# hjsuh94/irs_mpc

Hardware: AMD Instinct MI355X
Metric: rollouts*timesteps/s (randomized-smoothing pass) + iLQR-iters/s (higher is better)
Workload: dtype f32; 1 GPU; planar_hand quasi-dynamic contact, zero-order-B smoothing, step QP solved exactly (dual active-set method) -- the metric's config; T=50, N_per_gpu=10000, N_total=10000, mode=ZERO_ORDER_B, contact_solver=exact, samples=supplied, resident in HBM (f32), parallelism=samples sharded over 1 GPU(s), 1 all-reduce of (T,P) f64 per step

## Files before the change

### irs_mpc_amd/csrc/smooth_ug.hip

```cpp
#include "smooth_common.hpp"

namespace {

#ifndef IRS_UG_SWEEPS
#define IRS_UG_SWEEPS 6
#endif
#ifndef IRS_UG_PDAS
#define IRS_UG_PDAS 4
#endif
#ifndef IRS_UG_BLOCK
#define IRS_UG_BLOCK 512
#endif
constexpr int kUgBlock = IRS_UG_BLOCK;
constexpr int kUgSweeps = IRS_UG_SWEEPS;
constexpr int kUgPdas = IRS_UG_PDAS;
constexpr int kUgTabStride = 76;
#ifndef IRS_UG_NOM_ROUNDS
#define IRS_UG_NOM_ROUNDS 2
#endif
constexpr int kUgNomRounds = IRS_UG_NOM_ROUNDS;
constexpr int kUgRing = 128;

template <class Model>
struct alignas(16) UgLds {
    static constexpr int NC = Model::NC, n = Model::NX, m = Model::NU;
    float tab[1 << NC][kUgTabStride];
    float W[NC][NC];
    float invw[NC];
    float Wd[NC];
    float r0[NC];
    float phi[NC];
    float C[m][NC];
    float JD[n][NC];
    float Jc[NC][n];
    float Dinv[n];
    float Db0[n];
    float DK[m];
    float q[n];
};

__device__ __forceinline__ float ug_uniform(float v) {
    return __int_as_float(__builtin_amdgcn_readfirstlane(__float_as_int(v)));
}

template <int NC>
struct UgUni {
    float W[NC * (NC + 1) / 2];
    float invw[NC];
    float r0[NC];
    __device__ __forceinline__ float w(int i, int j) const {
        return i <= j ? W[i * NC - i * (i - 1) / 2 + (j - i)] : W[j * NC - j * (j - 1) / 2 + (i - j)];
    }
};

template <class Model>
__device__ __forceinline__ unsigned ug_lookup(const UgLds<Model>& S, unsigned a, const float* x, float tol, float* v,
                                              float* tau) {
    constexpr int NC = Model::NC;
    static_assert(NC == 8, "table entries are 8 x 8");
    const float4* e = reinterpret_cast<const float4*>(&S.tab[a][0]);
    float4 g4[2 * NC + 2];
#pragma unroll
    for (int c = 0; c < 2 * NC + 2; ++c) g4[c] = e[c];
    const unsigned ap = __float_as_uint(S.tab[a][72]);
    tau[0] = g4[16].x; tau[1] = g4[16].y; tau[2] = g4[16].z; tau[3] = g4[16].w;
    tau[4] = g4[17].x; tau[5] = g4[17].y; tau[6] = g4[17].z; tau[7] = g4[17].w;
#pragma unroll
    for (int i = 0; i < NC; ++i) v[i] = tau[i] * tol;
#pragma unroll
    for (int c = 0; c < NC; ++c) {
        const float4 lo = g4[2 * c], hi = g4[2 * c + 1];
        v[0] = fmaf(lo.x, x[c], v[0]); v[1] = fmaf(lo.y, x[c], v[1]);
        v[2] = fmaf(lo.z, x[c], v[2]); v[3] = fmaf(lo.w, x[c], v[3]);
        v[4] = fmaf(hi.x, x[c], v[4]); v[5] = fmaf(hi.y, x[c], v[5]);
        v[6] = fmaf(hi.z, x[c], v[6]); v[7] = fmaf(hi.w, x[c], v[7]);
    }
    return ap;
}

template <class Model>
__device__ __forceinline__ float ug_rhs(const UgUni<Model::NC>& U, const UgLds<Model>& S, const float* du, float* r) {
    constexpr int NC = Model::NC, m = Model::NU;
#pragma unroll
    for (int c = 0; c < NC; ++c) r[c] = U.r0[c];
#pragma unroll
    for (int j = 0; j < m; ++j) {
        const float4 lo = *reinterpret_cast<const float4*>(&S.C[j][0]);
        const float4 hi = *reinterpret_cast<const float4*>(&S.C[j][4]);
        r[0] = fmaf(lo.x, du[j], r[0]); r[1] = fmaf(lo.y, du[j], r[1]);
        r[2] = fmaf(lo.z, du[j], r[2]); r[3] = fmaf(lo.w, du[j], r[3]);
        r[4] = fmaf(hi.x, du[j], r[4]); r[5] = fmaf(hi.y, du[j], r[5]);
        r[6] = fmaf(hi.z, du[j], r[6]); r[7] = fmaf(hi.w, du[j], r[7]);
    }
    float scale = 1e-30f;
#pragma unroll
    for (int c = 0; c < NC; ++c) scale = fmaxf(scale, fabsf(r[c]));
    return 1e-6f * scale;
}

template <class Model>
__device__ __forceinline__ bool ug_try(const UgUni<Model::NC>& U, const UgLds<Model>& S, const float* r, float tolv,
                                       float* lam, unsigned& a_out, int diag = 0) {
    constexpr int NC = Model::NC;
    float g[NC];
#pragma unroll
    for (int i = 0; i < NC; ++i) { lam[i] = 0.f; g[i] = r[i]; }
#pragma unroll 2
    for (int sw = 0; sw < ((diag & 64) ? 0 : kUgSweeps); ++sw) {
#pragma unroll
        for (int i = 0; i < NC; ++i) {
            const float nw = fmaxf(fmaf(-g[i], U.invw[i], lam[i]), 0.f);
            const float dl = nw - lam[i];
            lam[i] = nw;
#pragma unroll
            for (int j = 0; j < NC; ++j) g[j] = fmaf(U.w(j, i), dl, g[j]);
        }
    }
    unsigned a = 0u;
#pragma unroll
    for (int i = 0; i < NC; ++i) a |= (lam[i] > 0.f) ? (1u << i) : 0u;
    bool done = (diag & 32) != 0;
    for (int it = 0; it < kUgPdas; ++it) {
        float v[NC], tau[NC];
        const unsigned ap = ug_lookup<Model>(S, a, r, tolv, v, tau);
        unsigned bad = 0u;
#pragma unroll
        for (int i = NC - 1; i >= 0; --i) bad = __builtin_amdgcn_alignbit(bad, __float_as_uint(v[i]), 31);
        if (!done) {
            if (bad == 0u) {
#pragma unroll
                for (int i = 0; i < NC; ++i) lam[i] = fmaf(-tau[i], v[i], v[i]);
                done = true;
            }
            a = ap ^ bad;
        }
        if (__all(done)) break;
    }
    a_out = a;
    return done;
}

template <class Model>
__device__ __forceinline__ void ug_full(const UgLds<Model>& S, const float* r, float tolv, unsigned a, float* lam,
                                        int cap = 4 * Model::NC) {
    constexpr int NC = Model::NC;
    constexpr float kBig = 3.0e38f, piv_rel = 1e-5f;
    float g[NC];
    bool valid = false;
    for (int round = 0; round < 3; ++round) {
        if (__all(valid)) break;
        float v[NC], tau[NC];
        const unsigned ap = ug_lookup<Model>(S, a, r, 0.f, v, tau);
        if (!valid) {
            unsigned negb = 0u;
#pragma unroll
            for (int i = 0; i < NC; ++i) {
                const bool in = tau[i] == 0.f;
                negb |= (in && !(v[i] > 0.f)) ? (1u << i) : 0u;
                lam[i] = in ? v[i] : 0.f;
                g[i] = in ? 0.f : v[i];
            }
            valid = negb == 0u;
            a = ap & ~negb;
        }
    }
    if (!valid) {
        a = 0u;
#pragma unroll
        for (int i = 0; i < NC; ++i) { lam[i] = 0.f; g[i] = r[i]; }
    }
    int p = -1;
    bool done = false;
    for (int it = 0; it < cap; ++it) {
        if (!done && p < 0) {
            float vmin = kBig;
            int c = 0;
#pragma unroll
            for (int i = 0; i < NC; ++i) {
                const float vv = ((a >> i) & 1u) ? kBig : g[i];
                if (vv < vmin) { vmin = vv; c = i; }
            }
            if (vmin >= -tolv) done = true;
            else p = c;
        }
        if (__all(done)) break;
        const int pp = (done || p < 0) ? 0 : p;
        float wp[NC], u[NC], tau[NC];
        {
            const float4 lo = *reinterpret_cast<const float4*>(&S.W[pp][0]);
            const float4 hi = *reinterpret_cast<const float4*>(&S.W[pp][4]);
            wp[0] = lo.x; wp[1] = lo.y; wp[2] = lo.z; wp[3] = lo.w;
            wp[4] = hi.x; wp[5] = hi.y; wp[6] = hi.z; wp[7] = hi.w;
        }
        ug_lookup<Model>(S, a, wp, 0.f, u, tau);
        const float wpp = S.Wd[pp];
        float gp = 0.f, zp = 0.f;
#pragma unroll
        for (int i = 0; i < NC; ++i) {
            const bool isp = i == pp;
            gp = isp ? g[i] : gp;
            zp = isp ? u[i] : zp;
        }
        const bool full_ok = zp > piv_rel * wpp;
        const float t2 = full_ok ? -gp * irs_rcp_fast(zp) : kBig;
        float rho[NC], qv[NC];
        float t1 = kBig;
#pragma unroll
        for (int i = 0; i < NC; ++i) {
            rho[i] = fmaf(tau[i], u[i], -u[i]);
            qv[i] = rho[i] > 0.f ? lam[i] * irs_rcp_fast(rho[i]) : kBig;
            t1 = fminf(t1, qv[i]);
        }
        int kb = 0;
#pragma unroll
        for (int i = NC - 1; i >= 0; --i) kb = (qv[i] == t1) ? i : kb;
        const float tmin = fminf(t1, t2);
        if (!done && !(tmin < kBig)) done = true;
        const float tt = done ? 0.f : tmin;
#pragma unroll
        for (int i = 0; i < NC; ++i) {
            g[i] = fmaf(tt * tau[i], u[i], g[i]);
            lam[i] = fmaxf(fmaf(-tt, rho[i], lam[i]) + ((i == pp) ? tt : 0.f), 0.f);
        }
        if (!done) {
            const bool full = t2 <= t1;
            if (full) {
                a |= 1u << pp;
                p = -1;
            } else {
                a &= ~(1u << kb);
#pragma unroll
                for (int i = 0; i < NC; ++i) lam[i] = (i == kb) ? 0.f : lam[i];
            }
        }
    }
}

template <class Model>
__device__ __forceinline__ void ug_build_entry(UgLds<Model>& S, unsigned a, int half) {
    constexpr int NC = Model::NC;
    constexpr float piv_rel = 1e-5f;
    float M_[NC][NC], inv[NC], W[NC][NC];
    bool act[NC];
#pragma unroll
    for (int i = 0; i < NC; ++i) {
        act[i] = ((a >> i) & 1u) != 0u;
#pragma unroll
        for (int j = 0; j < NC; ++j) W[i][j] = S.W[i][j];
#pragma unroll
        for (int j = 0; j <= i; ++j) M_[i][j] = W[i][j];
    }
    unsigned ap = 0u;
#pragma unroll
    for (int j = 0; j < NC; ++j) {
        const float dj = M_[j][j];
        const bool ok = act[j] && dj > piv_rel * W[j][j];
        act[j] = ok;
        ap |= ok ? (1u << j) : 0u;
        inv[j] = ok ? irs_rcp_fast(dj) : 0.f;
#pragma unroll
        for (int i = j + 1; i < NC; ++i) M_[j][i] = M_[i][j] * inv[j];
#pragma unroll
        for (int i = j + 1; i < NC; ++i)
#pragma unroll
            for (int k = j + 1; k <= i; ++k) M_[i][k] = M_[i][k] - M_[j][i] * M_[k][j];
    }
    float* e = &S.tab[a][0];
    for (int cc = 0; cc < NC / 2; ++cc) {
        const int c = half * (NC / 2) + cc;
        float y[NC];
#pragma unroll
        for (int j = 0; j < NC; ++j) {
            float v = (act[j] && j == c) ? -1.f : 0.f;
#pragma unroll
            for (int k = 0; k < j; ++k) v = v - M_[k][j] * y[k];
            y[j] = v;
        }
#pragma unroll
        for (int j = NC - 1; j >= 0; --j) {
            float v = y[j] * inv[j];
#pragma unroll
            for (int i = j + 1; i < NC; ++i) v = v - M_[j][i] * y[i];
            y[j] = v;
        }
        float col[NC];
#pragma unroll
        for (int i = 0; i < NC; ++i) {
            float s = (i == c) ? 1.f : 0.f;
#pragma unroll
            for (int j = 0; j < NC; ++j) s = fmaf(W[i][j], y[j], s);
            col[i] = act[i] ? y[i] : s;
        }
        *reinterpret_cast<float4*>(e + 8 * c) = make_float4(col[0], col[1], col[2], col[3]);
        *reinterpret_cast<float4*>(e + 8 * c + 4) = make_float4(col[4], col[5], col[6], col[7]);
    }
    if (half == 0) {
        *reinterpret_cast<float4*>(e + 64) = make_float4(act[0] ? 0.f : 1.f, act[1] ? 0.f : 1.f, act[2] ? 0.f : 1.f, act[3] ? 0.f : 1.f);
        *reinterpret_cast<float4*>(e + 68) = make_float4(act[4] ? 0.f : 1.f, act[5] ? 0.f : 1.f, act[6] ? 0.f : 1.f, act[7] ? 0.f : 1.f);
        e[72] = __uint_as_float(ap);
    }
}

struct UgNomLds {
    double J[8][7];
    double q[7], Dinv[7], b[7];
};

template <class Model>
__device__ __forceinline__ double ug_nominal_geometry(const SmoothArgs& a, UgNomLds& L, int t, int lane) {
    constexpr int NC = Model::NC, n = Model::NX, m = Model::NU;
    double x64[n], u64[m], q[n], Dinv[n], b[n], J[NC][n], phi[NC];
#pragma unroll
    for (int i = 0; i < n; ++i) x64[i] = a.x_trj[(size_t)t * n + i];
#pragma unroll
    for (int j = 0; j < m; ++j) u64[j] = a.u_trj[(size_t)t * m + j];
    Model::template assemble<double>(a.p, x64, u64, q, Dinv, b, J, phi);
    if (lane == 0) {
#pragma unroll
        for (int c = 0; c < NC; ++c)
#pragma unroll
            for (int k = 0; k < n; ++k) L.J[c][k] = J[c][k];
#pragma unroll
        for (int k = 0; k < n; ++k) { L.q[k] = q[k]; L.Dinv[k] = Dinv[k]; L.b[k] = b[k]; }
    }
    double rr = 0.0;
#pragma unroll
    for (int c = 0; c < NC; ++c) {
        double s = phi[c];
#pragma unroll
        for (int k = 0; k < n; ++k) s -= J[c][k] * (b[k] * Dinv[k]);
        rr = (lane == c) ? s : rr;
    }
    wave_sync();
    return rr;
}

template <class Model>
__device__ __forceinline__ void ug_nominal(const SmoothArgs& a, const UgUni<Model::NC>& U, const UgLds<Model>& S,
                                           UgNomLds& L, double rr, int t, int lane) {
    constexpr int NC = Model::NC, n = Model::NX, m = Model::NU;
    static_assert(NC == 8 && n <= 8, "lane (i,k) = 8 i + k owns entry (i,k) of the 8 x 8 dual Hessian");
    float du0[m], r32[NC], lam32[NC];
#pragma unroll
    for (int j = 0; j < m; ++j) du0[j] = 0.f;
    const float tolv = ug_rhs<Model>(U, S, du0, r32);
    unsigned am = 0u;
    if (!ug_try<Model>(U, S, r32, tolv, lam32, am)) ug_full<Model>(S, r32, tolv, am, lam32);
    unsigned set = 0u;
#pragma unroll
    for (int i = 0; i < NC; ++i) set |= (lam32[i] > 0.f) ? (1u << i) : 0u;
    set = (unsigned)__builtin_amdgcn_readfirstlane((int)set);
    {
        const int li = lane >> 3, lk = lane & 7;
        double w = 0.0;
#pragma unroll
        for (int kk = 0; kk < n; ++kk) w += L.J[li][kk] * L.Dinv[kk] * L.J[lk][kk];
        double scale = 1e-300;
#pragma unroll
        for (int c = 0; c < NC; ++c) scale = fmax(scale, fabs(__shfl(rr, c, 64)));
        const double tol64 = 1e-10 * scale;
        double lamd = 0.0;
        bool settled = false;
        for (int corr = 0; corr < 8 && !settled; ++corr) {
            double M = w, Lf = 0.0;
            unsigned eff = 0u;
            double invd[NC];
#pragma unroll
            for (int j = 0; j < NC; ++j) {
                const double dj = __shfl(M, 9 * j, 64), wjj = __shfl(w, 9 * j, 64);
                const bool ok = ((set >> j) & 1u) && dj > 1e-7 * wjj;
                eff |= ok ? (1u << j) : 0u;
                invd[j] = ok ? 1.0 / dj : 0.0;
                const double Mij = __shfl(M, 8 * li + j, 64), Mkj = __shfl(M, 8 * lk + j, 64);
                if (lk == j && li > j) Lf = Mij * invd[j];
                if (li > j && lk > j) M -= Mij * invd[j] * Mkj;
            }
            const bool mine = lane < NC && ((eff >> lane) & 1u);
            double y = mine ? -rr : 0.0;
#pragma unroll
            for (int j = 0; j < NC; ++j) {
                const double yj = __shfl(y, j, 64);
                const double Lij = __shfl(Lf, 8 * (lane & 7) + j, 64);
                if (lane < NC && lane > j) y -= Lij * yj;
            }
            double invme = 0.0;
#pragma unroll
            for (int j = 0; j < NC; ++j) invme = (lane == j) ? invd[j] : invme;
            y *= invme;
#pragma unroll
            for (int j = NC - 1; j >= 0; --j) {
                const double yj = __shfl(y, j, 64);
                const double Lji = __shfl(Lf, 8 * j + (lane & 7), 64);
                if (lane < j) y -= Lji * yj;
            }
            lamd = mine ? y : 0.0;
            double pr = w * __shfl(lamd, lk, 64);
            pr += __shfl_xor(pr, 1, 64);
            pr += __shfl_xor(pr, 2, 64);
            pr += __shfl_xor(pr, 4, 64);
            const double sl = rr + __shfl(pr, 8 * (lane & 7), 64);
            const bool neg = lane < NC && mine && !(lamd > 0.0);
            const bool viol = lane < NC && !mine && sl < -tol64;
            const unsigned negb = (unsigned)(__ballot(neg) & 0xffull), violb = (unsigned)(__ballot(viol) & 0xffull);
            if ((negb | violb) == 0u) settled = true;
            else set = (eff & ~negb) | violb;
        }
        double f = 0.0;
        if (settled) {
            double acc = 0.0;
#pragma unroll
            for (int c = 0; c < NC; ++c) acc += L.J[c][lane < n ? lane : 0] * __shfl(lamd, c, 64);
            if (lane < n) f = L.q[lane] + L.Dinv[lane] * (acc - L.b[lane]);
        } else if (lane < n) {
            float acc = -S.Db0[lane];
#pragma unroll
            for (int c = 0; c < NC; ++c) acc = fmaf(S.JD[lane][c], lam32[c], acc);
            f = (double)(S.q[lane] + acc);
        }
        if (lane < n)
            __hip_atomic_store(a.fnom + (size_t)t * n + Model::perm(lane), f, __ATOMIC_RELAXED, __HIP_MEMORY_SCOPE_AGENT);
    }
}

#ifdef IRS_UG_STAMPS
constexpr int kUgStampSlots = 12, kUgStampWgs = 2048;
__device__ unsigned long long ug_stamps[kUgStampWgs * kUgStampSlots];
#define UG_STAMP(slot)                                                                          \
    do {                                                                                        \
        if ((threadIdx.x & 63) == 0) {                                                          \
            const int wg_ = blockIdx.y * gridDim.x + blockIdx.x;                                \
            if (wg_ < kUgStampWgs && ((slot) < 8 ? threadIdx.x == 0 : true))                    \
                ug_stamps[wg_ * kUgStampSlots + (slot)] = __builtin_amdgcn_s_memtime();         \
        }                                                                                       \
    } while (0)
#else
#define UG_STAMP(slot) do {} while (0)
#endif

template <class Model, int MODE, bool RNG, bool FUSE>
__global__ __launch_bounds__(kUgBlock) void smooth_ug_kernel(SmoothArgs a) {
    using TR = SmoothTraits<Model, MODE>;
    constexpr int n = TR::n, m = TR::m, P = TR::P, NC = Model::NC;
    constexpr int BLOCK = kUgBlock, NW = BLOCK / 64;
    static_assert(TR::Z0 == n && NC == 8 && m == 4, "u-only smoothing of an 8-row contact model with 4 commands");
    static_assert(P < kBlock, "the hand-off's group reduction");
    constexpr int NG = m * (m + 1) / 2;
    constexpr int PI = TR::FIRST_B ? 1 : NG + m * NC + m;
    constexpr int PPI = irs_reduce_pad(TR::FIRST_B ? n * m : PI);
    constexpr int QE = m + 1;
    __shared__ UgLds<Model> S;
    __shared__ UgNomLds nomL;
    __shared__ float ring_all[NW * kUgRing * QE];
    __shared__ float red[NW * (PPI > TR::PP ? PPI : TR::PP)];
    __shared__ float toti[PPI];
    __shared__ unsigned hist[TR::FIRST_B ? (1 << NC) : 1];
    __shared__ double red64[TR::NGRP * P];
    __shared__ double tot[P];
    __shared__ FinalizeLds<Model, MODE> fin;
    __shared__ int s_ticket;

    const int t = blockIdx.y, blk = blockIdx.x, tid = threadIdx.x;
    const int lane = tid & 63, wave = tid >> 6;

    UG_STAMP(0);
    const bool nominal_wave = blk == 0 && wave == NW - 1;
    double nom_r = 0.0;
    if (nominal_wave && !(a.diag & 2)) nom_r = ug_nominal_geometry<Model>(a, nomL, t, lane);
    if (wave == 0) {
        float xb[n], ub[m], q[n], Dinv[n], b0[n], J[NC][n], phi[NC];
#pragma unroll
        for (int i = 0; i < n; ++i) xb[i] = (float)a.x_trj[(size_t)t * n + i];
#pragma unroll
        for (int j = 0; j < m; ++j) ub[j] = (float)a.u_trj[(size_t)t * m + j];
        Model::template assemble<float>(a.p, xb, ub, q, Dinv, b0, J, phi);
        if (lane == 0) {
#pragma unroll
            for (int i = 0; i < NC; ++i) {
                S.phi[i] = phi[i];
#pragma unroll
                for (int k = 0; k < n; ++k) S.Jc[i][k] = J[i][k];
            }
#pragma unroll
            for (int k = 0; k < n; ++k) { S.Db0[k] = b0[k] * Dinv[k]; S.q[k] = q[k]; S.Dinv[k] = Dinv[k]; }
#pragma unroll
            for (int j = 0; j < m; ++j) S.DK[j] = Dinv[Model::act(j)] * Model::template stiffness<float>(a.p, j);
        }
    }
    if constexpr (TR::FIRST_B) {
        for (int q = tid; q < (1 << NC); q += BLOCK) hist[q] = 0u;
    }
    __syncthreads();
    if (tid < NC * NC) {
        const int i = tid / NC, j = tid % NC, hi = i > j ? i : j, lo = i > j ? j : i;
        float w = (S.Jc[hi][0] * S.Dinv[0]) * S.Jc[lo][0];
#pragma unroll
        for (int k = 1; k < n; ++k) w = w + (S.Jc[hi][k] * S.Dinv[k]) * S.Jc[lo][k];
        S.W[i][j] = w;
        if (i == j) {
            S.Wd[i] = w;
            S.invw[i] = (float)kContactPgsOmega * irs_rcp_fast(w);
        }
    } else if (tid < NC * NC + NC) {
        const int i = tid - NC * NC;
        float ri = S.phi[i];
#pragma unroll
        for (int k = 0; k < n; ++k) ri = ri - S.Jc[i][k] * S.Db0[k];
        S.r0[i] = ri;
    } else if (tid < 2 * NC * NC + NC) {
        const int e = tid - (NC * NC + NC), k = e / NC, c = e % NC;
        if (k < n) S.JD[k][c] = S.Jc[c][k] * S.Dinv[k];
    } else if (tid < 2 * NC * NC + NC + m * NC) {
        const int e = tid - (2 * NC * NC + NC), j = e / NC, c = e % NC;
        S.C[j][c] = (S.Jc[c][Model::act(j)] * S.Dinv[Model::act(j)]) * Model::template stiffness<float>(a.p, j);
    }
    __syncthreads();
    UG_STAMP(1);
    if (!(a.diag & 4))
        for (int e = tid; e < 2 * (1 << NC); e += BLOCK) ug_build_entry<Model>(S, (unsigned)(e >> 1), e & 1);
    __syncthreads();

    UG_STAMP(2);
    UgUni<NC> U;
    {
        int q = 0;
#pragma unroll
        for (int i = 0; i < NC; ++i)
#pragma unroll
            for (int j = i; j < NC; ++j) U.W[q++] = S.W[i][j];
#pragma unroll
        for (int i = 0; i < NC; ++i) { U.invw[i] = S.invw[i]; U.r0[i] = S.r0[i]; }
    }

    float acc[PPI];
#pragma unroll
    for (int i = 0; i < PPI; ++i) acc[i] = 0.f;

    if (nominal_wave && !(a.diag & 2)) ug_nominal<Model>(a, U, S, nomL, nom_r, t, lane);
    if (nominal_wave) UG_STAMP(8);
    if (!(a.diag & 8)) {
        const int V = a.nblk * NW;
        const int me = nominal_wave ? V - 1 : (blk == 0 ? wave : blk * NW - 1 + wave);
        const int nblocks = (a.N + 63) / 64;
        int round = nominal_wave ? kUgNomRounds : 0;
        auto block_of = [&](int k) { return k < kUgNomRounds ? k * (V - 1) + me : kUgNomRounds * (V - 1) + (k - kUgNomRounds) * V + me; };
        float* ring = ring_all + wave * (kUgRing * QE);
        int qhead = 0, qtail = 0;
        int bk = block_of(round);
        float du_next[m];
#pragma unroll
        for (int j = 0; j < m; ++j) du_next[j] = 0.f;
        auto request = [&](int block) {
            if constexpr (!RNG) {
                if (block < nblocks) {
                    const int sidx = block * 64 + lane;
                    const size_t row = (size_t)t * a.N + (sidx < a.N ? sidx : a.N - 1);
                    load_row<m>(a.du + row * m, du_next);
                }
            }
        };
        request(bk);
        while (true) {
            const bool fresh = bk < nblocks;
            const int pending = qtail - qhead;
            const bool flush = pending >= 64 || (!fresh && pending > 0);
            if (!fresh && !flush) break;
            float du[m], r[NC], lam[NC];
            bool on, fin_ = true;
            if (flush) {
                __builtin_amdgcn_fence(__ATOMIC_RELEASE, "wavefront");
                __builtin_amdgcn_wave_barrier();
                __builtin_amdgcn_fence(__ATOMIC_ACQUIRE, "wavefront");
                const int take = min(64, pending);
                on = lane < take;
                const int slot = (qhead + (on ? lane : 0)) & (kUgRing - 1);
#pragma unroll
                for (int j = 0; j < m; ++j) du[j] = ring[slot * QE + j];
                const unsigned wm = __float_as_uint(ring[slot * QE + m]);
                const float tolv = ug_rhs<Model>(U, S, du, r);
                ug_full<Model>(S, r, tolv, wm, lam, (a.diag & 128) ? 8 : ((a.diag & 256) ? 12 : 4 * NC));
                qhead += take;
            } else {
                const int sidx = bk * 64 + lane;
                on = sidx < a.N;
                if constexpr (RNG) {
                    const unsigned long long gidx = a.sample_offset + (unsigned long long)sidx;
#pragma unroll
                    for (int j = n / 4; j < (n + m + 3) / 4; ++j) {
                        float g4[4];
                        philox_normal4(gidx, (unsigned)t, (unsigned)j, a.iter, a.seed, g4);
#pragma unroll
                        for (int c = 0; c < 4; ++c) {
                            const int idx = 4 * j + c;
                            if (idx >= n && idx < n + m) du[idx - n] = __fmul_rn(g4[c], a.std[idx]);
                        }
                    }
                } else {
#pragma unroll
                    for (int j = 0; j < m; ++j) du[j] = du_next[j];
                    request(block_of(round + 1));
                }
                const float tolv = ug_rhs<Model>(U, S, du, r);
                unsigned mask = 0u;
                fin_ = ug_try<Model>(U, S, r, tolv, lam, mask, a.diag);
                if (a.diag & 16) fin_ = true;
                const bool hard = on && !fin_;
                const unsigned long long bal = __ballot(hard);
                if (hard) {
                    const int slot = (qtail + __popcll(bal & ((1ull << lane) - 1ull))) & (kUgRing - 1);
#pragma unroll
                    for (int j = 0; j < m; ++j) ring[slot * QE + j] = du[j];
                    ring[slot * QE + m] = __uint_as_float(mask);
                }
                qtail += __popcll(bal);
                bk = block_of(++round);
            }
            const bool use = on && fin_;
            bool nonfinite = false;
#pragma unroll
            for (int j = 0; j < m; ++j) nonfinite = nonfinite || irs_nonfinite_bits(du[j]);
            if constexpr (TR::FIRST_B) {
                unsigned I = 0u;
#pragma unroll
                for (int i = 0; i < NC; ++i) I |= (lam[i] * S.Wd[i] > (float)kContactActiveTol) ? (1u << i) : 0u;
                if (use) __hip_atomic_fetch_add(&hist[I], 1u, __ATOMIC_RELAXED, __HIP_MEMORY_SCOPE_WORKGROUP);
                if (on && nonfinite) acc[0] = irs_poison();
            } else {
                float zz[m];
#pragma unroll
                for (int j = 0; j < m; ++j) zz[j] = use ? du[j] : 0.f;
                int q = 0;
#pragma unroll
                for (int i = 0; i < m; ++i)
#pragma unroll
                    for (int j = i; j < m; ++j) { acc[q] = fmaf(zz[i], zz[j], acc[q]); ++q; }
#pragma unroll
                for (int i = 0; i < m; ++i)
#pragma unroll
                    for (int c = 0; c < NC; ++c) { acc[q] = fmaf(zz[i], lam[c], acc[q]); ++q; }
#pragma unroll
                for (int i = 0; i < m; ++i) { acc[q] += zz[i]; ++q; }
                if (on && nonfinite) acc[0] = irs_poison();
            }
        }
    }

    UG_STAMP(3);
    if (blk == 0 && wave == 1) UG_STAMP(9);
    if constexpr (TR::FIRST_B) {
        __syncthreads();
        unsigned poison_bits = __float_as_uint(acc[0]);
        asm volatile("" : "+v"(poison_bits));
#pragma unroll
        for (int i = 0; i < PPI; ++i) acc[i] = 0.f;
        for (int I = tid; I < (1 << NC); I += BLOCK) {
            const unsigned cnt = hist[I];
            if (cnt == 0u) continue;
            const float* e = &S.tab[I][0];
            const unsigned ap = __float_as_uint(e[72]);
            float Y[NC][m];
#pragma unroll
            for (int i = 0; i < NC; ++i) {
                const bool in = ((ap >> i) & 1u) != 0u;
#pragma unroll
                for (int c = 0; c < m; ++c) {
                    float s = 0.f;
#pragma unroll
                    for (int j = 0; j < NC; ++j) s = fmaf(e[8 * j + i], S.Jc[j][Model::act(c)], s);
                    Y[i][c] = in ? -s : 0.f;
                }
            }
#pragma unroll
            for (int k = 0; k < n; ++k)
#pragma unroll
                for (int c = 0; c < m; ++c) {
                    float s = 0.f;
#pragma unroll
                    for (int i = 0; i < NC; ++i) s = fmaf(S.Jc[i][k], Y[i][c], s);
                    const float Bkc = (k == Model::act(c) ? 1.f : 0.f) - S.Dinv[k] * s;
                    acc[Model::perm(k) * m + c] += (float)cnt * Bkc;
                }
        }
        if ((poison_bits & 0x7f800000u) == 0x7f800000u) acc[0] = irs_poison();
        block_reduce_lds<P, NW>(acc, red);
    } else {
        block_reduce_lds<PI, NW>(acc, red);
        __syncthreads();
        for (int q = tid; q < PI; q += BLOCK) {
            float s = red[q];
#pragma unroll
            for (int w = 1; w < NW; ++w) s += red[w * PPI + q];
            toti[q] = s;
        }
        __syncthreads();
        float out = 0.f;
        if (tid < P) {
            if (tid < NG) out = toti[tid];
            else if (tid < NG + m * n) {
                const int i = (tid - NG) / n, kext = (tid - NG) % n;
                int k = 0, jact = -1;
#pragma unroll
                for (int kk = 0; kk < n; ++kk) k = (Model::perm(kk) == kext) ? kk : k;
#pragma unroll
                for (int j = 0; j < m; ++j) jact = (Model::act(j) == k) ? j : jact;
                float s = -S.Db0[k] * toti[NG + m * NC + i];
                for (int c = 0; c < NC; ++c) s = fmaf(S.JD[k][c], toti[NG + i * NC + c], s);
                if (jact >= 0) {
                    const int lo = i < jact ? i : jact, hi = i < jact ? jact : i;
                    s = fmaf(S.DK[jact], toti[lo * m - lo * (lo - 1) / 2 + (hi - lo)], s);
                }
                out = s;
            } else {
                out = toti[NG + m * NC + (tid - NG - m * n)];
            }
        }
        __syncthreads();
        for (int q = tid; q < NW * TR::PP; q += BLOCK) red[q] = 0.f;
        __syncthreads();
        if (tid < P) red[tid] = out;
    }
    UG_STAMP(4);
    smooth_finish<Model, MODE, FUSE, BLOCK, true>(a, red, red64, tot, fin, s_ticket, t, blk, tid, a.fnom + (size_t)t * n);
    UG_STAMP(5);
}

template <class Model, int MODE>
void ug_launch_m(const SmoothArgs& a, bool rng, bool fuse, hipStream_t st) {
    dim3 grid(a.nblk, a.T), block(kUgBlock);
    if (rng) {
        if (fuse) hipLaunchKernelGGL((smooth_ug_kernel<Model, MODE, true, true>), grid, block, 0, st, a);
        else hipLaunchKernelGGL((smooth_ug_kernel<Model, MODE, true, false>), grid, block, 0, st, a);
    } else {
        if (fuse) hipLaunchKernelGGL((smooth_ug_kernel<Model, MODE, false, true>), grid, block, 0, st, a);
        else hipLaunchKernelGGL((smooth_ug_kernel<Model, MODE, false, false>), grid, block, 0, st, a);
    }
}

}

#ifdef IRS_UG_STAMPS
extern "C" int irs_debug_ug_stamps(unsigned long long* host_out, int n_wgs) {
    if (n_wgs > kUgStampWgs) n_wgs = kUgStampWgs;
    return (int)hipMemcpyFromSymbol(host_out, HIP_SYMBOL(ug_stamps), (size_t)n_wgs * kUgStampSlots * sizeof(unsigned long long));
}
#endif

bool irs_smooth_ug_supported(int model, int mode) {
    const char* e = getenv("IRS_UG");
    if (e != nullptr && atoi(e) == 0) return false;
    return model == IRS_MODEL_PLANAR_HAND_EXACT && (mode == IRS_SMOOTH_ZERO_ORDER_B || mode == IRS_SMOOTH_FIRST_ORDER);
}

int irs_smooth_ug_nblk(int T, int N) {
    static int cus = 0;
    if (cus == 0) {
        hipDeviceProp_t prop;
        int dev = 0;
        cus = (hipGetDevice(&dev) == hipSuccess && hipGetDeviceProperties(&prop, dev) == hipSuccess)
                  ? prop.multiProcessorCount : 256;
        if (cus < 1) cus = 256;
    }
    const int nblocks = (N + 63) / 64, NW = kUgBlock / 64;
    int nb = cus / (T < 1 ? 1 : T);
    if (nb < 1) nb = 1;
    const int by_work = (nblocks + 1 + NW - 1) / NW;
    if (nb > by_work) nb = by_work;
    return nb < 1 ? 1 : nb;
}

int irs_smooth_ug_launch(int model, int mode, const SmoothArgs& a, bool rng, bool fuse, hipStream_t st) {
    if (model != IRS_MODEL_PLANAR_HAND_EXACT) return IRS_ERR_UNSUPPORTED;
    if (mode == IRS_SMOOTH_ZERO_ORDER_B) ug_launch_m<PlanarHandExactModel, IRS_SMOOTH_ZERO_ORDER_B>(a, rng, fuse, st);
    else if (mode == IRS_SMOOTH_FIRST_ORDER) ug_launch_m<PlanarHandExactModel, IRS_SMOOTH_FIRST_ORDER>(a, rng, fuse, st);
    else return IRS_ERR_UNSUPPORTED;
    return IRS_OK;
}
```

Baseline: 13.17 billion rollouts*timesteps/s.

## Hand off straggler active-set solves to quad-lane cooperative finishing

Once only a few lanes (at most 16) are still iterating in the full dual active-set loop, their state (lambda, g, active mask, pivot, tolerance) is staged to LDS. Each remaining sample is then finished by a quad of four lanes that each own two constraint rows, using DPP quad reductions for the min and pick steps. This targets wave divergence, where a whole wave waits on a few slow lanes doing serial 8-row work. It adds LDS staging, extra wave syncs and a per-wave stage buffer. A diag bit can disable the hand-off and another can force every sample down the hard path.

```diff
diff --git a/irs_mpc_amd/csrc/smooth_ug.hip b/irs_mpc_amd/csrc/smooth_ug.hip
--- a/irs_mpc_amd/csrc/smooth_ug.hip
+++ b/irs_mpc_amd/csrc/smooth_ug.hip
@@ -140,9 +140,112 @@
     return done;
 }
 
+__device__ __forceinline__ float ug_row_ratio(float tau, float u, float lam, float& rho) {
+    rho = fmaf(tau, u, -u);
+    return rho > 0.f ? lam * irs_rcp_fast(rho) : 3.0e38f;
+}
+__device__ __forceinline__ void ug_row_step(float tt, float tau, float u, float rho, bool isp, float& g, float& lam) {
+    g = fmaf(tt * tau, u, g);
+    lam = fmaxf(fmaf(-tt, rho, lam) + (isp ? tt : 0.f), 0.f);
+}
+
+constexpr int kUgStageSlots = 16;
+constexpr int kUgStageStride = 20;
+
+template <int CTRL>
+__device__ __forceinline__ int ug_quad_perm(int v) {
+    return __builtin_amdgcn_update_dpp(0, v, CTRL, 0xf, 0xf, true);
+}
+__device__ __forceinline__ float ug_quad_min(float v) {
+    v = fminf(v, __int_as_float(ug_quad_perm<0xB1>(__float_as_int(v))));
+    return fminf(v, __int_as_float(ug_quad_perm<0x4E>(__float_as_int(v))));
+}
+__device__ __forceinline__ int ug_quad_min(int v) {
+    v = min(v, ug_quad_perm<0xB1>(v));
+    return min(v, ug_quad_perm<0x4E>(v));
+}
+__device__ __forceinline__ float ug_quad_pick(float v) {
+    v = v + __int_as_float(ug_quad_perm<0xB1>(__float_as_int(v)));
+    return v + __int_as_float(ug_quad_perm<0x4E>(__float_as_int(v)));
+}
+
 template <class Model>
+__device__ __forceinline__ void ug_finish_quads(const UgLds<Model>& S, float* stage, int nslots, int it, int cap, int lane) {
+    constexpr int NC = Model::NC;
+    static_assert(NC == 8, "four lanes of two rows each");
+    constexpr float kBig = 3.0e38f, piv_rel = 1e-5f;
+    const int q = lane >> 2, h = lane & 3, i0 = 2 * h, i1 = 2 * h + 1;
+    const bool have = q < nslots;
+    float* slot = stage + (have ? q : 0) * kUgStageStride;
+    const float2 l2 = *reinterpret_cast<const float2*>(slot + i0);
+    const float2 g2 = *reinterpret_cast<const float2*>(slot + NC + i0);
+    const float2 ap2 = *reinterpret_cast<const float2*>(slot + 2 * NC);
+    const float tolv = slot[2 * NC + 2];
+    float lam0 = l2.x, lam1 = l2.y, g0 = g2.x, g1 = g2.y;
+    unsigned a = __float_as_uint(ap2.x);
+    int p = __float_as_int(ap2.y);
+    bool done = !have;
+    for (; it < cap; ++it) {
+        if (!done && p < 0) {
+            const float vv0 = ((a >> i0) & 1u) ? kBig : g0, vv1 = ((a >> i1) & 1u) ? kBig : g1;
+            const float vmin = ug_quad_min(fminf(vv0, vv1));
+            const int c = ug_quad_min(vv0 == vmin ? i0 : (vv1 == vmin ? i1 : NC)) & (NC - 1);
+            if (vmin >= -tolv) done = true;
+            else p = c;
+        }
+        if (__all(done)) break;
+        const int pp = (done || p < 0) ? 0 : p;
+        float wp[NC];
+        {
+            const float4 lo = *reinterpret_cast<const float4*>(&S.W[pp][0]);
+            const float4 hi = *reinterpret_cast<const float4*>(&S.W[pp][4]);
+            wp[0] = lo.x; wp[1] = lo.y; wp[2] = lo.z; wp[3] = lo.w;
+            wp[4] = hi.x; wp[5] = hi.y; wp[6] = hi.z; wp[7] = hi.w;
+        }
+        const float* e = &S.tab[a][0];
+        float2 col[NC];
+#pragma unroll
+        for (int c = 0; c < NC; ++c) col[c] = *reinterpret_cast<const float2*>(e + 8 * c + i0);
+        const float2 tau2 = *reinterpret_cast<const float2*>(e + 64 + i0);
+        const float wpp = S.Wd[pp];
+        float u0 = tau2.x * 0.f, u1 = tau2.y * 0.f;
+#pragma unroll
+        for (int c = 0; c < NC; ++c) {
+            u0 = fmaf(col[c].x, wp[c], u0);
+            u1 = fmaf(col[c].y, wp[c], u1);
+        }
+        const bool mine = (pp >> 1) == h, odd = (pp & 1) != 0;
+        const float gp = ug_quad_pick(mine ? (odd ? g1 : g0) : 0.f);
+        const float zp = ug_quad_pick(mine ? (odd ? u1 : u0) : 0.f);
+        const bool full_ok = zp > piv_rel * wpp;
+        const float t2 = full_ok ? -gp * irs_rcp_fast(zp) : kBig;
+        float rho0, rho1;
+        const float qv0 = ug_row_ratio(tau2.x, u0, lam0, rho0), qv1 = ug_row_ratio(tau2.y, u1, lam1, rho1);
+        const float t1 = ug_quad_min(fminf(qv0, qv1));
+        const int kb = ug_quad_min(qv0 == t1 ? i0 : (qv1 == t1 ? i1 : NC)) & (NC - 1);
+        const float tmin = fminf(t1, t2);
+        if (!done && !(tmin < kBig)) done = true;
+        const float tt = done ? 0.f : tmin;
+        ug_row_step(tt, tau2.x, u0, rho0, i0 == pp, g0, lam0);
+        ug_row_step(tt, tau2.y, u1, rho1, i1 == pp, g1, lam1);
+        if (!done) {
+            if (t2 <= t1) {
+                a |= 1u << pp;
+                p = -1;
+            } else {
+                a &= ~(1u << kb);
+                lam0 = (i0 == kb) ? 0.f : lam0;
+                lam1 = (i1 == kb) ? 0.f : lam1;
+            }
+        }
+    }
+    if (have) *reinterpret_cast<float2*>(slot + i0) = make_float2(lam0, lam1);
+}
+
+template <class Model, bool STAGED = false>
 __device__ __forceinline__ void ug_full(const UgLds<Model>& S, const float* r, float tolv, unsigned a, float* lam,
-                                        int cap = 4 * Model::NC) {
+                                        int cap = 4 * Model::NC, bool on = true, bool one_lane = true,
+                                        float* stage = nullptr, int lane = 0) {
     constexpr int NC = Model::NC;
     constexpr float kBig = 3.0e38f, piv_rel = 1e-5f;
     float g[NC];
@@ -170,8 +273,10 @@
         for (int i = 0; i < NC; ++i) { lam[i] = 0.f; g[i] = r[i]; }
     }
     int p = -1;
-    bool done = false;
-    for (int it = 0; it < cap; ++it) {
+    bool done = STAGED ? !on : false;
+    int it = 0;
+    unsigned long long hand = 0ull;
+    for (; it < cap; ++it) {
         if (!done && p < 0) {
             float vmin = kBig;
             int c = 0;
@@ -183,7 +288,13 @@
             if (vmin >= -tolv) done = true;
             else p = c;
         }
-        if (__all(done)) break;
+        if constexpr (STAGED) {
+            const unsigned long long live = __ballot(!done);
+            if (live == 0ull) break;
+            if (!one_lane && __popcll(live) <= kUgStageSlots) { hand = live; break; }
+        } else {
+            if (__all(done)) break;
+        }
         const int pp = (done || p < 0) ? 0 : p;
         float wp[NC], u[NC], tau[NC];
         {
@@ -207,8 +318,7 @@
         float t1 = kBig;
 #pragma unroll
         for (int i = 0; i < NC; ++i) {
-            rho[i] = fmaf(tau[i], u[i], -u[i]);
-            qv[i] = rho[i] > 0.f ? lam[i] * irs_rcp_fast(rho[i]) : kBig;
+            qv[i] = ug_row_ratio(tau[i], u[i], lam[i], rho[i]);
             t1 = fminf(t1, qv[i]);
         }
         int kb = 0;
@@ -218,10 +328,7 @@
         if (!done && !(tmin < kBig)) done = true;
         const float tt = done ? 0.f : tmin;
 #pragma unroll
-        for (int i = 0; i < NC; ++i) {
-            g[i] = fmaf(tt * tau[i], u[i], g[i]);
-            lam[i] = fmaxf(fmaf(-tt, rho[i], lam[i]) + ((i == pp) ? tt : 0.f), 0.f);
-        }
+        for (int i = 0; i < NC; ++i) ug_row_step(tt, tau[i], u[i], rho[i], i == pp, g[i], lam[i]);
         if (!done) {
             const bool full = t2 <= t1;
             if (full) {
@@ -231,6 +338,28 @@
                 a &= ~(1u << kb);
 #pragma unroll
                 for (int i = 0; i < NC; ++i) lam[i] = (i == kb) ? 0.f : lam[i];
+            }
+        }
+    }
+    if constexpr (STAGED) {
+        if (hand != 0ull) {
+            const bool mine = ((hand >> lane) & 1ull) != 0ull;
+            float* slot = stage + __popcll(hand & ((1ull << lane) - 1ull)) * kUgStageStride;
+            wave_sync();
+            if (mine) {
+                *reinterpret_cast<float4*>(slot) = make_float4(lam[0], lam[1], lam[2], lam[3]);
+                *reinterpret_cast<float4*>(slot + 4) = make_float4(lam[4], lam[5], lam[6], lam[7]);
+                *reinterpret_cast<float4*>(slot + 8) = make_float4(g[0], g[1], g[2], g[3]);
+                *reinterpret_cast<float4*>(slot + 12) = make_float4(g[4], g[5], g[6], g[7]);
+                *reinterpret_cast<float4*>(slot + 16) = make_float4(__uint_as_float(a), __int_as_float(p), tolv, 0.f);
+            }
+            wave_sync();
+            ug_finish_quads<Model>(S, stage, __popcll(hand), it, cap, lane);
+            wave_sync();
+            if (mine) {
+                const float4 lo = *reinterpret_cast<const float4*>(slot), hi = *reinterpret_cast<const float4*>(slot + 4);
+                lam[0] = lo.x; lam[1] = lo.y; lam[2] = lo.z; lam[3] = lo.w;
+                lam[4] = hi.x; lam[5] = hi.y; lam[6] = hi.z; lam[7] = hi.w;
             }
         }
     }
@@ -451,6 +580,7 @@
     __shared__ UgLds<Model> S;
     __shared__ UgNomLds nomL;
     __shared__ float ring_all[NW * kUgRing * QE];
+    __shared__ __attribute__((aligned(16))) float stage_all[NW * kUgStageSlots * kUgStageStride];
     __shared__ float red[NW * (PPI > TR::PP ? PPI : TR::PP)];
     __shared__ float toti[PPI];
     __shared__ unsigned hist[TR::FIRST_B ? (1 << NC) : 1];
@@ -577,7 +707,8 @@
                 for (int j = 0; j < m; ++j) du[j] = ring[slot * QE + j];
                 const unsigned wm = __float_as_uint(ring[slot * QE + m]);
                 const float tolv = ug_rhs<Model>(U, S, du, r);
-                ug_full<Model>(S, r, tolv, wm, lam, (a.diag & 128) ? 8 : ((a.diag & 256) ? 12 : 4 * NC));
+                ug_full<Model, true>(S, r, tolv, wm, lam, (a.diag & 128) ? 8 : ((a.diag & 256) ? 12 : 4 * NC), on,
+                                     (a.diag & 512) != 0, stage_all + wave * (kUgStageSlots * kUgStageStride), lane);
                 qhead += take;
             } else {
                 const int sidx = bk * 64 + lane;
@@ -603,6 +734,7 @@
                 unsigned mask = 0u;
                 fin_ = ug_try<Model>(U, S, r, tolv, lam, mask, a.diag);
                 if (a.diag & 16) fin_ = true;
+                if (a.diag & 1024) fin_ = false;
                 const bool hard = on && !fin_;
                 const unsigned long long bal = __ballot(hard);
                 if (hard) {
```

New measurement: 13.65 billion rollouts*timesteps/s (median of 5 runs). +3.6%, better.
